# jedisct1/zig-lz4

Measured on AMD Instinct MI355X. Metric: GiB/s uncompressed, block compress+decompress, higher is better.
Workload: dtype u8

## Files before the change

### zig-lz4_amd/csrc/zlz4_compress_fast.hip

```cpp
#include <cstdlib>

#include "zlz4_device.hpp"
#include "zlz4_launch.hpp"

#ifdef ZLZ4_STAMPS
__device__ unsigned long long g_zlz4_stamps[24];
#define STAMP_DECL unsigned long long st_acc[24] = {0,0,0,0,0,0,0,0,0,0,0,0,0,0,0,0,0,0,0,0,0,0,0,0}; unsigned long long st_last = __builtin_amdgcn_s_memtime();
#define STAMP(i) do { unsigned long long st_now; __builtin_amdgcn_sched_barrier(0); \
                      asm volatile("s_memtime %0\n\ts_waitcnt lgkmcnt(0)" : "=s"(st_now) :: "memory"); \
                      __builtin_amdgcn_sched_barrier(0); st_acc[i] += st_now - st_last; st_last = st_now; } while (0)
#define STAMP_COUNT(i) do { st_acc[i] += 1; } while (0)
#define STAMP_FLUSH do { if (lane == 0) for (int st_k = 0; st_k < 24; st_k++) atomicAdd(&g_zlz4_stamps[st_k], st_acc[st_k]); } while (0)
#else
#define STAMP_DECL
#define STAMP(i)
#define STAMP_COUNT(i)
#define STAMP_FLUSH
#endif

namespace zlz4 {

__device__ __forceinline__ uint32_t hash4(uint32_t seq) { return (seq * kHashMul) >> 20; }

__device__ __forceinline__ uint32_t skip_sum(uint32_t x) {
    const uint32_t q = x >> 6, r = x & 63u;
    return 32u * q * (q - 1u) + q * r;
}

__device__ __forceinline__ int64_t emit_last_literals(uint8_t *dst, uint32_t dst_len, uint32_t op,
                                                       const uint8_t *lit_src, uint32_t lit, uint32_t lane) {
    if (lit == 0) return (int64_t)op;
    const uint32_t nle = ext_len_bytes(lit);
    if ((uint64_t)op + 1u + nle + lit > dst_len) return kErrOutputTooSmall;
    if (lane == 0) dst[op] = (uint8_t)((lit >= 15u ? 15u : lit) << 4);
    if (lit >= 15u) write_ext_len(dst + op + 1u, lit, lane);
    copy_bytes(dst + op + 1u + nle, lit_src, lit, lane);
    return (int64_t)(op + 1u + nle + lit);
}

__device__ __forceinline__ uint32_t extend_match(const uint8_t *__restrict__ src, uint32_t m_pos, uint32_t m_cand,
                                                 uint32_t mlen, uint32_t match_limit, uint32_t src_size,
                                                 uint32_t lane) {
    const uint32_t ip0 = m_pos + kMinMatch, mt0 = m_cand + kMinMatch;
    for (;;) {
        const uint32_t p = ip0 + mlen + lane * 16u;
        uint32_t n = 0;
        if (p < match_limit) n = (match_limit - p) < 16u ? (match_limit - p) : 16u;
        uint32_t d = 0;
        if (n > 0) {
            const uint32_t q = mt0 + mlen + lane * 16u;
            if (p + 16u <= src_size) {
                d = first_diff16(ld128(src + p), ld128(src + q));
                if (d > n) d = n;
            } else {
                while (d < n && src[p + d] == src[q + d]) d++;
            }
        }
        const uint64_t stop = ballot(d < 16u);
        if (stop) {
            const uint32_t sl = first_lane(stop);
            return mlen + sl * 16u + rdlane(d, sl);
        }
        mlen += 1024u;
    }
}

template <typename T, int kTag, bool kSeed = false>
__global__ __launch_bounds__(256) void k_compress_fast(
    const uint8_t *__restrict__ d_in, const uint64_t *__restrict__ d_in_off,
    const uint32_t *__restrict__ d_in_len, uint8_t *__restrict__ d_out,
    const uint64_t *__restrict__ d_out_off, const uint32_t *__restrict__ d_out_cap,
    int64_t *__restrict__ d_result, uint32_t nblocks, uint32_t acceleration, uint32_t max_in_len,
    const uint32_t *d_table_in, const uint32_t *__restrict__ d_table_idx, uint32_t *d_table_out) {
    extern __shared__ __attribute__((aligned(16))) uint8_t lds_raw[];
    const uint32_t lane = threadIdx.x & 63u;
    const uint32_t wave_in_wg = threadIdx.x >> 6;
    const uint32_t blk = rfl(blockIdx.x * (blockDim.x >> 6) + wave_in_wg);
    if (blk >= nblocks) return;
    typedef __attribute__((address_space(3))) volatile T lds_entry;
    typedef __attribute__((address_space(3))) volatile uint8_t lds_tag;
    lds_entry *table = (lds_entry *)lds_raw + wave_in_wg * 4096u;
    lds_tag *tags = (lds_tag *)lds_raw + (blockDim.x >> 6) * 4096u * (uint32_t)sizeof(T) + wave_in_wg * 4096u;
    constexpr uint32_t kPosMask = kTag == 2 ? 0x00FFFFFFu : 0xFFFFFFFFu;

    const uint8_t *src = d_in + d_in_off[blk];
    uint8_t *dst = d_out + d_out_off[blk];
    const uint32_t src_size = rfl(d_in_len[blk]);
    const uint32_t dst_len = rfl(d_out_cap[blk]);

    int64_t res;
    if (src_size > kMaxInput) {
        res = kErrInputTooLarge;
    } else if (src_size > max_in_len) {
        res = kErrInvalidState;
    } else if (src_size == 0) {
        res = 0;
    } else if (src_size < kMfLimit + 1u) {
        res = emit_last_literals(dst, dst_len, 0, src, src_size, lane);
    } else {
        if constexpr (kSeed) {
            const uint32_t L = src_size - kMfLimit;
            const uint32_t tix = d_table_idx ? rfl(d_table_idx[blk]) : blk;
            const u32x4 *seed4 = reinterpret_cast<const u32x4 *>(d_table_in + (uint64_t)tix * 4096u);
            for (uint32_t k = lane; k < 1024u; k += 64u) {
                const u32x4 v = seed4[k];
                uint32_t e[4] = {v.x < L ? v.x : 0u, v.y < L ? v.y : 0u, v.z < L ? v.z : 0u, v.w < L ? v.w : 0u};
                if (kTag == 2) {
                    for (int q = 0; q < 4; q++)
                        if (e[q]) e[q] |= ((ld32(src + e[q]) * kHashMul) >> 12 & 0xFFu) << 24;
                }
                for (int q = 0; q < 4; q++) table[4u * k + q] = (T)e[q];
            }
            __builtin_amdgcn_fence(__ATOMIC_RELEASE, "wavefront");
        } else {
        {
            u32x4 z = {0, 0, 0, 0};
            u32x4 *t4 = reinterpret_cast<u32x4 *>(lds_raw) + wave_in_wg * (4096u * sizeof(T) / 16u);
            const uint32_t n16 = 4096u * sizeof(T) / 16u;
            for (uint32_t k = lane; k < n16; k += 64u) t4[k] = z;
        }
        }
        const uint32_t accel = acceleration < 1u ? 1u : (acceleration > 65537u ? 65537u : acceleration);
        const uint32_t cbase = accel > 64u ? accel : 64u;
        const uint32_t s_cbase = skip_sum(cbase);
        const uint32_t L = src_size - kMfLimit;
        const uint32_t match_limit = src_size - kLastLiterals;
        const uint64_t lane_bit = 1ull << lane;
        const uint64_t lanes_below = lane_bit - 1ull;

        uint32_t anchor = 0, op = 0;
        uint32_t F0 = 1;
        bool has_ins = false;
        bool failed = false;
        STAMP_DECL
        STAMP(0);

        uint32_t guard = 0;

        constexpr bool kRing = sizeof(T) == 2;
        uint32_t rpos = 0x80000000u + 4u * lane;
        uint32_t r0 = 0, r1 = 0, r2 = 0;
        uint32_t ring_lim = 0;
        if constexpr (kRing) asm volatile("v_mov_b32 %0, %1" : "=v"(ring_lim) : "s"(src_size - 4u));
        auto ring_q = [&](uint32_t q) -> uint32_t { return q < ring_lim ? q : ring_lim; };
        auto ring_sel = [&](uint32_t A, uint32_t &ja) -> uint32_t {
            uint32_t rel = rfl(A - rpos);
            if (rel >= 256u) {
                const bool reload = rel >= 512u;
                const uint32_t nb = reload ? (A & ~127u) + 4u * lane : rpos + 256u;
                asm volatile("s_waitcnt vmcnt(0)\n\t"
                             "s_cmpk_lt_u32 %[rel], 0x200\n\t"
                             "s_cbranch_scc1 1f\n\t"
                             "global_load_dword %[r0], %[q0], %[src]\n\t"
                             "global_load_dword %[r1], %[q1], %[src]\n\t"
                             "s_waitcnt vmcnt(0)\n\t"
                             "s_branch 2f\n"
                             "1:\n\t"
                             "v_mov_b32 %[r0], %[r1]\n\t"
                             "v_mov_b32 %[r1], %[r2]\n"
                             "2:\n\t"
                             "global_load_dword %[r2], %[q2], %[src]"
                             : [r0] "+v"(r0), [r1] "+v"(r1), [r2] "+v"(r2)
                             : [rel] "s"(rel), [q0] "v"(ring_q(nb)), [q1] "v"(ring_q(nb + 256u)), [q2] "v"(ring_q(nb + 512u)),
                               [src] "s"(src)
                             : "scc", "memory");
                rpos = nb;
                rel = reload ? A & 127u : rel - 256u;
            }
            ja = ((rel & ~3u) + (((A & 3u) + lane) & ~3u)) & 0xFFu;
            return lane >= (rel >> 2) ? r0 : r1;
        };
#define ZLZ4_SEL_DWORD(sel, ja, K) ((uint32_t)__builtin_amdgcn_ds_bpermute((int)add_wrap_byte<4u * (K)>(ja), (int)(sel)))
        auto ring_fwd = [&](uint32_t sel, uint32_t ja, uint32_t A, uint32_t &hi4) -> u32x4 {
            const uint32_t sh = (A + lane) & 3u;
            const uint32_t w0 = (uint32_t)__builtin_amdgcn_ds_bpermute((int)ja, (int)sel);
            const uint32_t w1 = ZLZ4_SEL_DWORD(sel, ja, 1), w2 = ZLZ4_SEL_DWORD(sel, ja, 2), w3 = ZLZ4_SEL_DWORD(sel, ja, 3);
            hi4 = ZLZ4_SEL_DWORD(sel, ja, 4);
            return u32x4{__builtin_amdgcn_alignbyte(w1, w0, sh), __builtin_amdgcn_alignbyte(w2, w1, sh),
                         __builtin_amdgcn_alignbyte(w3, w2, sh), __builtin_amdgcn_alignbyte(hi4, w3, sh)};
        };
        auto ring_fwd2 = [&](uint32_t sel, uint32_t ja, uint32_t A, uint32_t hi4, u32x4 &f2, u32x4 &f3) {
            const uint32_t sh = (A + lane) & 3u;
            const uint32_t w5 = ZLZ4_SEL_DWORD(sel, ja, 5), w6 = ZLZ4_SEL_DWORD(sel, ja, 6), w7 = ZLZ4_SEL_DWORD(sel, ja, 7);
            const uint32_t w8 = ZLZ4_SEL_DWORD(sel, ja, 8), w9 = ZLZ4_SEL_DWORD(sel, ja, 9), w10 = ZLZ4_SEL_DWORD(sel, ja, 10);
            const uint32_t w11 = ZLZ4_SEL_DWORD(sel, ja, 11), w12 = ZLZ4_SEL_DWORD(sel, ja, 12);
            f2 = u32x4{__builtin_amdgcn_alignbyte(w5, hi4, sh), __builtin_amdgcn_alignbyte(w6, w5, sh),
                       __builtin_amdgcn_alignbyte(w7, w6, sh), __builtin_amdgcn_alignbyte(w8, w7, sh)};
            f3 = u32x4{__builtin_amdgcn_alignbyte(w9, w8, sh), __builtin_amdgcn_alignbyte(w10, w9, sh),
                       __builtin_amdgcn_alignbyte(w11, w10, sh), __builtin_amdgcn_alignbyte(w12, w11, sh)};
        };
#undef ZLZ4_SEL_DWORD
        u32x4 fwd_pf = {0, 0, 0, 0};
        uint32_t sel_pf = 0, ja_pf = 0, hi4_pf = 0;
        uint32_t pf_anchor = 0xFFFFFFFFu;
        while (F0 < L) {
            if (++guard > src_size) { failed = true; break; }
            int32_t ub = -1;

            if (accel == 1u && F0 == anchor + 1u && has_ins && (uint64_t)anchor + 192u < L) {
              bool moved = false;
              bool to_generic = false;
              for (;;) {
                const uint32_t A = anchor;
                const uint32_t pos = A + lane;
                if (kRing && pf_anchor != A) {
                    sel_pf = ring_sel(A, ja_pf);
                    fwd_pf = ring_fwd(sel_pf, ja_pf, A, hi4_pf);
                }
                const uint32_t sel = sel_pf, ja = ja_pf, hi4 = hi4_pf;
                const u32x4 fwd = (kRing || pf_anchor == A) ? fwd_pf : ld128(src + pos);
                const uint32_t prod = fwd.x * kHashMul;
                const uint32_t h = prod >> 20;
                const uint32_t tg = (prod >> 12) & 0xFFu;
                const uint32_t mine = kTag == 2 ? (pos | (tg << 24)) : (uint32_t)(T)pos;
                STAMP(1);
                STAMP_COUNT(16);
                uint32_t told = tg;
                const uint32_t old_e = table[h];
                if (kTag == 1) told = tags[h];
                if (kTag == 2) told = old_e >> 24;
                const uint32_t old = old_e & kPosMask;
                uint64_t okm = ballot(old > 0) & ballot(old + kMaxDist >= pos);
                if (kSeed) okm &= ballot(old < pos);
                if (kTag != 0) okm &= ballot(told == tg);
                const bool old_ok = in_mask(okm);
                u32x4 cold = {0, 0, 0, 0};
                if (old_ok) cold = ld128(src + old);
                constexpr bool kGuess2 = sizeof(T) == 4;
                const uint32_t old12 = kGuess2 ? shfl(old, (lane + 12u) & 63u) : 0u;
                const bool pred2 = kGuess2 && old_ok && lane < 52u && old12 == old + 12u;
                u32x4 f2 = {0, 0, 0, 0}, c2 = f2, f3 = f2, c3 = f2;
                if (pred2) {
                    if (!kRing) { f2 = ld128(src + pos + 16u); f3 = ld128(src + pos + 32u); }
                    c2 = ld128(src + old + 16u); c3 = ld128(src + old + 32u);
                }
                STAMP(3);
                table[h] = (T)mine;
                __builtin_amdgcn_fence(__ATOMIC_RELEASE, "wavefront");
                const uint32_t rb = table[h];
                uint64_t losers = ballot(rb != mine);
                uint64_t grp = lane_bit;
                while (losers) {
                    const uint32_t l = first_lane(losers);
                    const uint32_t hh = rdlane(h, l);
                    const uint64_t same = ballot(h == hh);
                    if (in_mask(same)) grp = same;
                    losers &= ~same;
                }
                STAMP(2);

                const uint64_t vom = okm & ballot(cold.x == fwd.x);
                const bool vo = in_mask(vom);
                uint32_t mlo;
                {
                    const uint32_t x1 = fwd.y ^ cold.y, x2 = fwd.z ^ cold.z, x3 = fwd.w ^ cold.w;
                    const uint32_t xs = x1 ? x1 : (x2 ? x2 : x3);
                    const uint32_t xbase = x1 ? 0u : (x2 ? 4u : 8u);
                    mlo = xs ? xbase + ((uint32_t)__builtin_ctz(xs) >> 3) : 12u;
                }
                const uint64_t need2m = vom & ballot(mlo == 12u);
                const bool need2 = in_mask(need2m);
                if (need2 && !pred2) {
                    if (!kRing) { f2 = ld128(src + pos + 16u); f3 = ld128(src + pos + 32u); }
                    c2 = ld128(src + old + 16u); c3 = ld128(src + old + 32u);
                }
                if (kRing && need2m) ring_fwd2(sel, ja, A, hi4, f2, f3);
                if (need2) {
                    const uint32_t d2 = first_diff16_sel(f2, c2);
                    mlo += d2 == 16u ? 16u + first_diff16_sel(f3, c3) : d2;
                }
                const uint64_t singm = ballot(lane_rank(grp) == 0u);
                const uint64_t lt44 = ballot(mlo < 44u);
                const uint64_t cfast = vom & lt44;
                const uint64_t nsing = ~singm;
                const uint64_t slow = (nsing & ~cfast) | (vom & ~lt44);
                const uint64_t fastm = cfast & singm;
                const uint64_t stopm = slow | (cfast & nsing);
                uint32_t J, S;
                {
                    const uint64_t mj = fastm >> lane, ms = stopm >> lane;
                    J = mj ? lane + (uint32_t)__builtin_ctzll(mj) : 64u;
                    S = ms ? lane + (uint32_t)__builtin_ctzll(ms) : 64u;
                }
                const uint32_t v_end = lane + kMinMatch + mlo;
                uint32_t mlo_e = mlo, off_e = pos - old;
                const uint32_t X = J < S ? J : S;
                const uint32_t Q = (mlo << 2) | (in_mask(nsing) ? 2u : 0u) | (vo ? 1u : 0u);
                uint32_t PK;
                {
                    const uint32_t ve_j = shfl(v_end, J & 63u);
                    const bool fastok = J < S;
                    PK = fastok ? (J | ((ve_j + 1u) << 6) | (ve_j >= 63u ? 0x80000000u : 0u)) : 0xFFFFFFFFu;
                }

                STAMP(6);
                uint32_t f = 1;
                uint32_t a = 0;
                uint64_t cov_acc = 0;
                bool continue_generic = false;
                const bool tight = dst_len - op < 512u;
                uint32_t a0 = a;
                uint64_t mm_run = 0;
                uint64_t E_run = 0;
                auto covered_now = [&]() -> uint64_t { return cov_acc | (E_run - (mm_run << 1)); };
                auto flush_run = [&]() {
                    STAMP(9); STAMP_COUNT(21);
                    const uint64_t covm = E_run - (mm_run << 1);
                    const uint64_t ends = (E_run | (1ull << a0) | 1ull) & (lanes_below | lane_bit);
                    const uint32_t pend = 63u - (uint32_t)__builtin_clzll(ends);
                    const bool is_m = in_mask(mm_run);
                    const uint32_t jlast = 63u - (uint32_t)__builtin_clzll(mm_run);
                    const uint64_t litmask = ((1ull << jlast) - 1ull) & ~((1ull << a0) - 1ull) & ~(covm | mm_run);
                    const bool is_lit = in_mask(litmask);
                    const uint64_t extm = mm_run & ballot(mlo_e >= 15u);
                    const uint64_t at_or_above = mm_run & ~lanes_below;
                    const uint32_t my_m = at_or_above ? (uint32_t)__builtin_ctzll(at_or_above) : lane;
                    const uint64_t ownm = ballot(my_m - pend >= 15u);
                    const uint32_t own_l = in_mask(ownm) ? 1u : 0u;
                    const uint64_t lextm = mm_run & ownm;
                    const uint32_t k = lane_rank(mm_run);
                    const uint32_t lb = lane_rank(litmask);
                    const uint32_t o1 = op + 3u * k + lb + 1u + lane_rank(extm) + lane_rank(lextm) + own_l;
                    if (is_lit) dst[o1] = (uint8_t)fwd.x;
                    if (is_m) {
                        const uint32_t lit_k = lane - pend;
                        uint8_t *tk = dst + (o1 - 1u - lit_k - own_l);
                        tk[0] = (uint8_t)(((lit_k < 15u ? lit_k : 15u) << 4) | (mlo_e < 15u ? mlo_e : 15u));
                        if (own_l) tk[1] = (uint8_t)(lit_k - 15u);
                        const uint16_t off16 = (uint16_t)off_e;
                        __builtin_memcpy(dst + o1, &off16, 2);
                        if (mlo_e >= 15u) dst[o1 + 2u] = (uint8_t)(mlo_e - 15u);
                    }
                    const uint32_t nm = (uint32_t)__popcll(mm_run);
                    op += 3u * nm + (uint32_t)__popcll(litmask) + (uint32_t)__popcll(extm) + (uint32_t)__popcll(lextm);
                    cov_acc |= covm;
                    mm_run = 0;
                    E_run = 0;
                    STAMP(10);
                };
                for (;;) {
                    if (mm_run == 0) a0 = a;
                    if (!tight && f < 64u) {
                        uint32_t t_pk, t_j;
#define ZLZ4_FAST_RUN_TRIP                                   \
                            "v_readlane_b32 %[pk], %[PK], %[f]\n\t" \
                            "s_cmp_lt_i32 %[pk], 0\n\t"      \
                            "s_cbranch_scc1 3f\n\t"          \
                            "s_lshr_b32 %[f], %[pk], 6\n\t"  \
                            "s_and_b32 %[j], %[pk], 63\n\t"  \
                            "s_bitset1_b64 %[mm], %[j]\n\t"  \
                            "s_sub_u32 %[a], %[f], 1\n\t"    \
                            "s_bitset1_b64 %[er], %[a]\n\t"
                        asm volatile(
                            "s_nop 3\n"
                            "1:\n\t"
                            ZLZ4_FAST_RUN_TRIP
                            ZLZ4_FAST_RUN_TRIP
                            "s_branch 1b\n"
                            "3:\n"
                            : [f] "+s"(f), [a] "+s"(a), [mm] "+s"(mm_run), [er] "+s"(E_run), [pk] "=&s"(t_pk), [j] "=&s"(t_j)
                            : [PK] "v"(PK)
                            : "scc");
#undef ZLZ4_FAST_RUN_TRIP
                        if (t_pk != 0xFFFFFFFFu) {
                            mm_run |= 1ull << (t_pk & 63u);
                            f = (t_pk >> 6) & 127u;
                            a = f - 1u;
                            if (a == 63u) E_run |= 1ull << 63;
                        }
                    }
                    STAMP(8);
                    if (f >= 64u) {
                        if (a == 0u) continue_generic = true;
                        break;
                    }

                    const uint32_t x = rdlane(X, f);
                    if (x >= 64u) {
                        if (a == 0u) continue_generic = true;
                        break;
                    }
                    const uint32_t q = rdlane(Q, x);
                    uint64_t pm = 0;
                    if (q & 2u) {
                        const uint64_t grp_x = (uint64_t)rdlane((uint32_t)grp, x) | ((uint64_t)rdlane((uint32_t)(grp >> 32), x) << 32);
                        pm = grp_x & ~covered_now() & ((1ull << x) - 1ull);
                    }
                    const uint32_t j = x;
                    const uint32_t m_pos = A + j;
                    uint32_t m_cand, mlen;
                    if (pm) {
                        const uint32_t pr = 63u - (uint32_t)__builtin_clzll(pm);
                        if (rdlane(fwd.x, pr) != rdlane(fwd.x, x)) { STAMP_COUNT(19); STAMP(9); f = x + 1u; continue; }
                        STAMP_COUNT(18);
                        m_cand = A + pr;
                        const uint64_t xa = ((uint64_t)(rdlane(fwd.z, j) ^ rdlane(fwd.z, pr)) << 32) | (rdlane(fwd.y, j) ^ rdlane(fwd.y, pr));
                        const uint32_t xb = rdlane(fwd.w, j) ^ rdlane(fwd.w, pr);
                        if (xa) mlen = (uint32_t)__builtin_ctzll(xa) >> 3;
                        else if (xb) mlen = 8u + ((uint32_t)__builtin_ctz(xb) >> 3);
                        else mlen = extend_match(src, m_pos, m_cand, 12u, match_limit, src_size, lane);
                    } else {
                        if (!(q & 1u)) { STAMP_COUNT(19); STAMP(9); f = x + 1u; continue; }
                        STAMP_COUNT(18);
                        mlen = q >> 2;
                        if (mlen < 44u && !tight) {
                            mm_run |= 1ull << j;
                            a = j + kMinMatch + mlen;
                            if (a < 64u) E_run |= 1ull << a;
                            STAMP(9);
                            if (a >= 64u) break;
                            f = a + 1u;
                            continue;
                        }
                        m_cand = rdlane(old, x);
                        if (mlen >= 44u) mlen = extend_match(src, m_pos, m_cand, 44u, match_limit, src_size, lane);
                    }
                    const uint32_t lit = j - a;
                    const uint32_t offset = m_pos - m_cand;
                    const uint32_t e = j + kMinMatch + mlen;
                    if (!tight && mlen < 270u) {
                        mlo_e = wrlane(mlen, j, mlo_e);
                        off_e = wrlane(offset, j, off_e);
                        mm_run |= 1ull << j;
                        if (e < 64u) E_run |= 1ull << e;
                        a = e;
                        STAMP(9);
                        if (e >= 64u) break;
                        f = e + 1u;
                        continue;
                    }
                    if (mm_run) flush_run();
                    const uint32_t nle = ext_len_bytes(lit), nme = ext_len_bytes(mlen);
                    const uint64_t seq_end = (uint64_t)op + 1u + nle + lit + 2u + nme;
                    if (seq_end > dst_len) { failed = true; break; }
                    if (lane == 0)
                        dst[op] = (uint8_t)(((lit >= 15u ? 15u : lit) << 4) | (mlen >= 15u ? 15u : mlen));
                    if (lit >= 15u) write_ext_len(dst + op + 1u, lit, lane);
                    uint8_t *o = dst + op + 1u + nle;
                    if (lane >= a && lane < j) o[lane - a] = (uint8_t)fwd.x;
                    o += lit;
                    if (lane < 2u) o[lane] = (uint8_t)(offset >> (8u * lane));
                    if (mlen >= 15u) write_ext_len(o + 2u, mlen, lane);
                    op = (uint32_t)seq_end;
                    {
                        const uint64_t upto_e = e >= 64u ? ~0ull : (1ull << e) - 1ull;
                        cov_acc |= upto_e & ~((2ull << j) - 1ull);
                    }
                    a = e;
                    if (e >= 64u) break;
                    f = e + 1u;
                }
                const bool next_win = !continue_generic && !failed && a != 0u && (uint64_t)A + a + 192u < L;
                if (next_win) {
                    pf_anchor = A + a;
                    if constexpr (kRing) {
                        sel_pf = ring_sel(pf_anchor, ja_pf);
                        fwd_pf = ring_fwd(sel_pf, ja_pf, pf_anchor, hi4_pf);
                    } else {
                        fwd_pf = ld128(src + pf_anchor + lane);
                    }
                }
                if (mm_run && !failed) flush_run();
                anchor = A + a;
                STAMP(4);
                const uint32_t f_end = continue_generic ? 64u : (a >= 64u ? 64u : a + 1u);
                const uint64_t ins = ~cov_acc & (f_end >= 64u ? ~0ull : (1ull << f_end) - 1ull);
                if (failed) break;
                const uint64_t gi = grp & ins;
                const bool put_mine = in_mask(ins) && (gi & ~lanes_below & ~lane_bit) == 0;
                if (put_mine || gi == 0) table[h] = (T)(put_mine ? mine : old_e);
                if (kTag == 1 && put_mine) tags[h] = (uint8_t)tg;
                __builtin_amdgcn_fence(__ATOMIC_RELEASE, "wavefront");
                STAMP(5);
                moved = anchor != A;
                to_generic = continue_generic;
                if (next_win) {
                    has_ins = true;
                    F0 = anchor + 1u;
                    continue;
                }
                break;
              }
                if (failed) break;
                if (!to_generic && moved) {
                    if (anchor < L) { has_ins = true; F0 = anchor + 1u; }
                    else { has_ins = false; F0 = L; }
                    continue;
                }
                if (to_generic) ub = 63;
            }

            bool found = false, bailed = false;
            uint32_t m_pos = 0, m_cand = 0, m_local = 0;
            bool m_local_done = false;
            for (;;) {
                const int32_t u = ub + (int32_t)lane;
                uint32_t pos, step_next;
                if (u <= 0) {
                    pos = (u < 0) ? F0 - 1u : F0;
                    step_next = accel;
                } else if (u == 1) {
                    pos = F0 + accel;
                    step_next = accel >> 6;
                } else {
                    const uint32_t x = cbase + (uint32_t)u - 1u;
                    pos = F0 + accel + skip_sum(x) - s_cbase;
                    step_next = x >> 6;
                }
                const bool is_probe = u >= 0;
                const bool bail = is_probe && ((uint64_t)pos + step_next > L);
                const uint64_t bail_mask = ballot(bail);
                const uint32_t nb = bail_mask ? first_lane(bail_mask) : 64u;
                const bool active = (lane < nb) && (is_probe || has_ins);

                const bool have16 = active && (pos + 16u <= src_size);
                u32x4 fwd = {0, 0, 0, 0};
                if (have16) fwd = ld128(src + pos);
                else if (active) fwd.x = ld32(src + pos);
                const uint32_t prod = fwd.x * kHashMul;
                const uint32_t h = prod >> 20;
                const uint32_t tg = (prod >> 12) & 0xFFu;
                const uint32_t mine = kTag == 2 ? (pos | (tg << 24)) : (uint32_t)(T)pos;

                uint32_t old_e = 0, rb = 0, told = tg;
                if (active) {
                    old_e = table[h];
                    if (kTag == 1) told = tags[h];
                    table[h] = (T)mine;
                }
                if (kTag == 2) told = old_e >> 24;
                const uint32_t old = old_e & kPosMask;
                __builtin_amdgcn_fence(__ATOMIC_RELEASE, "wavefront");
                if (active) rb = table[h];
                uint64_t losers = ballot(active && rb != mine);
                uint64_t grp = lane_bit;
                int32_t pred = -1;
                while (losers) {
                    const uint32_t l = first_lane(losers);
                    const uint32_t hh = rdlane(h, l);
                    const uint64_t same = ballot(active && h == hh);
                    if (active && h == hh) {
                        grp = same;
                        const uint64_t below = same & lanes_below;
                        pred = below ? 63 - (int32_t)__clzll((long long)below) : -1;
                    }
                    losers &= ~same;
                }
                const uint32_t pred_pos = shfl(pos, (uint32_t)(pred < 0 ? 0 : pred));
                const uint32_t cand = pred >= 0 ? pred_pos : old;

                bool valid = is_probe && active && cand > 0 && cand < pos && (cand + kMaxDist >= pos) &&
                             (kTag == 0 || pred >= 0 || told == tg);
                u32x4 cnd = {0, 0, 0, 0};
                if (valid) {
                    if (have16) cnd = ld128(src + cand); else cnd.x = ld32(src + cand);
                    valid = cnd.x == fwd.x;
                }
                const uint64_t valid_mask = ballot(valid);

                if (valid_mask) {
                    const uint32_t wl = first_lane(valid_mask);
                    if (active && lane > wl) table[h] = (T)old_e;
                    __builtin_amdgcn_fence(__ATOMIC_RELEASE, "wavefront");
                    const uint64_t upto = (2ull << wl) - 1ull;
                    if (active && lane <= wl && ((grp & upto & ~lanes_below & ~lane_bit) == 0)) {
                        table[h] = (T)mine;
                        if (kTag == 1) tags[h] = (uint8_t)tg;
                    }
                    uint32_t loc = 0;
                    bool loc_done = false;
                    if (lane == wl) {
                        const uint32_t lim = match_limit - (pos + kMinMatch);
                        if (have16) {
                            u32x4 a = fwd, b = cnd;
                            a.x = 0; b.x = 0;
                            loc = first_diff16(a, b) - 4u;
                            if (loc >= lim) { loc = lim; loc_done = true; }
                            else if (loc < 12u) loc_done = true;
                        }
                    }
                    m_pos = rdlane(pos, wl);
                    m_cand = rdlane(cand, wl);
                    m_local = rdlane(loc, wl);
                    m_local_done = rdlane((uint32_t)loc_done, wl) != 0;
                    found = true;
                    break;
                }
                if (bail_mask) {
                    if constexpr (kSeed) {
                        if (active && ((grp & ~lanes_below & ~lane_bit) == 0) && grp != lane_bit) table[h] = (T)mine;
                        __builtin_amdgcn_fence(__ATOMIC_RELEASE, "wavefront");
                    }
                    bailed = true; break;
                }
                if (active && ((grp & ~lanes_below & ~lane_bit) == 0)) {
                    if (grp != lane_bit) table[h] = (T)mine;
                    if (kTag == 1) tags[h] = (uint8_t)tg;
                }
                __builtin_amdgcn_fence(__ATOMIC_RELEASE, "wavefront");
                ub += 64;
            }
            if (bailed || !found) break;
            STAMP_COUNT(20);

            const uint32_t mlen = m_local_done ? m_local
                                               : extend_match(src, m_pos, m_cand, m_local, match_limit, src_size, lane);

            const uint32_t lit = m_pos - anchor;
            const uint32_t nle = ext_len_bytes(lit), nme = ext_len_bytes(mlen);
            const uint64_t seq_end = (uint64_t)op + 1u + nle + lit + 2u + nme;
            if (seq_end > dst_len) { failed = true; break; }
            if (lane == 0)
                dst[op] = (uint8_t)(((lit >= 15u ? 15u : lit) << 4) | (mlen >= 15u ? 15u : mlen));
            if (lit >= 15u) write_ext_len(dst + op + 1u, lit, lane);
            uint8_t *o = dst + op + 1u + nle;
            copy_bytes(o, src + anchor, lit, lane);
            o += lit;
            const uint32_t offset = m_pos - m_cand;
            if (lane < 2u) o[lane] = (uint8_t)(offset >> (8u * lane));
            if (mlen >= 15u) write_ext_len(o + 2u, mlen, lane);
            op = (uint32_t)seq_end;

            const uint32_t end = m_pos + kMinMatch + mlen;
            anchor = end;
            if (end < L) { has_ins = true; F0 = end + 1u; }
            else { has_ins = false; F0 = L; }
        }
        if constexpr (kRing) asm volatile("s_waitcnt vmcnt(0)" : "+v"(r2));
        if constexpr (kSeed) {
            if (!failed && has_ins && F0 >= L && lane == 0) {
                const uint32_t prod = ld32(src + anchor) * kHashMul;
                table[prod >> 20] = (T)(kTag == 2 ? (anchor | ((prod >> 12 & 0xFFu) << 24)) : anchor);
            }
        }
        res = failed ? kErrOutputTooSmall
                     : emit_last_literals(dst, dst_len, op, src + anchor, src_size - anchor, lane);
        STAMP(7);
        STAMP_FLUSH;
    }
    if constexpr (kSeed) {
        if (d_table_out) {
            const uint32_t tix = d_table_idx ? rfl(d_table_idx[blk]) : blk;
            const uint32_t *seed = d_table_in + (uint64_t)tix * 4096u;
            uint32_t *out = d_table_out + (uint64_t)blk * 4096u;
            const bool merged = src_size >= kMfLimit + 1u && src_size <= max_in_len && src_size <= kMaxInput && res >= 0;
            if (merged) {
                const uint32_t L = src_size - kMfLimit;
                __builtin_amdgcn_fence(__ATOMIC_RELEASE, "wavefront");
                for (uint32_t k = lane; k < 4096u; k += 64u) {
                    const uint32_t v = seed[k];
                    const uint32_t loaded = v < L ? v : 0u;
                    const uint32_t f = (uint32_t)table[k] & kPosMask;
                    out[k] = f != loaded ? f : v;
                }
            } else if (out != seed) {
                const u32x4 *s4 = reinterpret_cast<const u32x4 *>(seed);
                u32x4 *o4 = reinterpret_cast<u32x4 *>(out);
                for (uint32_t k = lane; k < 1024u; k += 64u) o4[k] = s4[k];
            }
        }
    }
    if (lane == 0) d_result[blk] = res;
}

__global__ __launch_bounds__(256) void k_load_dict(const uint8_t *__restrict__ d_dict, const uint64_t *__restrict__ d_dict_off,
                                                   const uint32_t *__restrict__ d_dict_len, uint32_t *__restrict__ d_tables,
                                                   int64_t *__restrict__ d_result, uint32_t ndicts) {
    __shared__ uint32_t t[4096];
    const uint32_t d = blockIdx.x;
    if (d >= ndicts) return;
    const uint32_t lane = threadIdx.x & 63u;
    const uint32_t len = d_dict_len[d];
    const uint32_t size = len < 65536u ? len : 65536u;
    const uint8_t *tail = d_dict + d_dict_off[d] + (len - size);
    for (uint32_t k = threadIdx.x; k < 4096u; k += blockDim.x) t[k] = 0;
    __syncthreads();
    if (size >= kMinMatch) {
        const uint32_t n = size - kMinMatch;
        for (uint32_t base = threadIdx.x - lane; base < n; base += blockDim.x) {
            const uint32_t i = base + lane;
            const bool act = i < n;
            const uint32_t h = act ? hash4(ld32(tail + i)) : 0xFFFFFFFFu;
            const uint32_t hr = shfl(h, lane + 1u);
            if (act && !(lane < 63u && hr == h)) atomicMax(&t[h], i);
        }
    }
    __syncthreads();
    uint32_t *out = d_tables + (uint64_t)d * 4096u;
    for (uint32_t k = threadIdx.x; k < 4096u; k += blockDim.x) out[k] = t[k];
    if (threadIdx.x == 0) d_result[d] = (int64_t)size;
}

}

extern "C" int zlz4_launch_compress_fast(hipStream_t stream, const uint8_t *d_in, const uint64_t *d_in_off,
                                         const uint32_t *d_in_len, uint8_t *d_out, const uint64_t *d_out_off,
                                         const uint32_t *d_out_cap, int64_t *d_result, uint32_t nblocks,
                                         uint32_t max_in_len, uint32_t acceleration) {
    if (nblocks == 0) return 0;
    static const uint32_t lds_pad = [] { const char *e = zlz4_tune_env("ZLZ4_TUNE_LDS_PAD"); return e ? (uint32_t)atoi(e) : 0u; }();
    static const uint32_t tune_wpw = [] { const char *e = zlz4_tune_env("ZLZ4_TUNE_WPW"); return e ? (uint32_t)atoi(e) : 0u; }();
    static const int tune_tag = [] { const char *e = zlz4_tune_env("ZLZ4_TUNE_TAG"); return e ? atoi(e) : -1; }();
#define ZLZ4_LAUNCH_FAST(KERN, T, TAG, WPW, LDS)                                                                      \
    hipLaunchKernelGGL((zlz4::KERN<T, TAG>), dim3((nblocks + (WPW) - 1) / (WPW)), dim3(64 * (WPW)), (LDS),              \
                       stream, d_in, d_in_off, d_in_len, d_out, d_out_off, d_out_cap, d_result, nblocks, acceleration,  \
                       max_in_len, nullptr, nullptr, nullptr)
    if (max_in_len <= 65536u + 11u) {
        const uint32_t wpw = (tune_wpw == 2 || tune_wpw == 4) ? tune_wpw : 1;
        if (tune_tag > 0) ZLZ4_LAUNCH_FAST(k_compress_fast, uint16_t, 1, wpw, wpw * (4096 * sizeof(uint16_t) + 4096) + lds_pad);
        else ZLZ4_LAUNCH_FAST(k_compress_fast, uint16_t, 0, wpw, wpw * 4096 * sizeof(uint16_t) + lds_pad);
    } else {
        const uint32_t wpw = (tune_wpw == 2) ? 2 : 1;
        if (tune_tag != 0 && max_in_len <= (1u << 24)) ZLZ4_LAUNCH_FAST(k_compress_fast, uint32_t, 2, wpw, wpw * 4096 * sizeof(uint32_t) + lds_pad);
        else ZLZ4_LAUNCH_FAST(k_compress_fast, uint32_t, 0, wpw, wpw * 4096 * sizeof(uint32_t) + lds_pad);
    }
#undef ZLZ4_LAUNCH_FAST
    return zlz4_launch_status();
}

extern "C" int zlz4_launch_compress_fast_continue(hipStream_t stream, const uint8_t *d_in, const uint64_t *d_in_off,
                                                  const uint32_t *d_in_len, uint8_t *d_out, const uint64_t *d_out_off,
                                                  const uint32_t *d_out_cap, const uint32_t *d_table_in,
                                                  const uint32_t *d_table_idx, uint32_t *d_table_out, int64_t *d_result,
                                                  uint32_t nblocks, uint32_t max_in_len, uint32_t acceleration) {
    if (nblocks == 0) return 0;
    static const int tune_tag = [] { const char *e = zlz4_tune_env("ZLZ4_TUNE_TAG"); return e ? atoi(e) : -1; }();
#define ZLZ4_LAUNCH_SEEDED(T, TAG)                                                                                      \
    hipLaunchKernelGGL((zlz4::k_compress_fast<T, TAG, true>), dim3(nblocks), dim3(64), 4096 * sizeof(T), stream, d_in,   \
                       d_in_off, d_in_len, d_out, d_out_off, d_out_cap, d_result, nblocks, acceleration, max_in_len,      \
                       d_table_in, d_table_idx, d_table_out)
    if (max_in_len <= 65536u + 11u) ZLZ4_LAUNCH_SEEDED(uint16_t, 0);
    else if (tune_tag != 0 && max_in_len <= (1u << 24)) ZLZ4_LAUNCH_SEEDED(uint32_t, 2);
    else ZLZ4_LAUNCH_SEEDED(uint32_t, 0);
#undef ZLZ4_LAUNCH_SEEDED
    return zlz4_launch_status();
}

extern "C" int zlz4_launch_load_dict(hipStream_t stream, const uint8_t *d_dict, const uint64_t *d_dict_off,
                                     const uint32_t *d_dict_len, uint32_t *d_tables, int64_t *d_result, uint32_t ndicts) {
    if (ndicts == 0) return 0;
    hipLaunchKernelGGL(zlz4::k_load_dict, dim3(ndicts), dim3(256), 0, stream, d_dict, d_dict_off, d_dict_len, d_tables,
                       d_result, ndicts);
    return zlz4_launch_status();
}

#ifdef ZLZ4_STAMPS
extern "C" int zlz4_debug_read_stamps(unsigned long long *out16, int reset) {
    if (hipMemcpyFromSymbol(out16, HIP_SYMBOL(g_zlz4_stamps), 24 * sizeof(unsigned long long)) != hipSuccess) return ZLZ4_ERR_DEVICE;
    if (reset) {
        unsigned long long z[24] = {0};
        if (hipMemcpyToSymbol(HIP_SYMBOL(g_zlz4_stamps), z, sizeof z) != hipSuccess) return ZLZ4_ERR_DEVICE;
    }
    return 0;
}
#endif
```

Baseline: 92.24.

## Stage compressor input ring window in LDS instead of register ds_bpermute gathers

Replaces the register-resident three-dword ring, which was read through many ds_bpermute cross-lane shuffles, with a 576-byte per-wave LDS ring buffer. Global loads are written into LDS, including a mirrored head region so reads can wrap, and forward windows are then read with one b32 plus one unaligned 128-bit LDS load per 16 bytes. This is meant to cut the number of permute instructions per window probe and to free VGPRs. In exchange it adds ds_writes, a wavefront fence and extra LDS per wave, and the static_assert is there to keep the occupancy granule count unchanged.

```diff
diff --git a/zig-lz4_amd/csrc/zlz4_compress_fast.hip b/zig-lz4_amd/csrc/zlz4_compress_fast.hip
--- a/zig-lz4_amd/csrc/zlz4_compress_fast.hip
+++ b/zig-lz4_amd/csrc/zlz4_compress_fast.hip
@@ -65,6 +65,10 @@
     }
 }
 
+constexpr uint32_t kRingBytes = 576;
+constexpr uint32_t kLdsGranule = 1280;
+static_assert(4096 * sizeof(uint16_t) + kRingBytes <= 7 * kLdsGranule, "the ring must fit the granules the u16 table already occupies");
+
 template <typename T, int kTag, bool kSeed = false>
 __global__ __launch_bounds__(256) void k_compress_fast(
     const uint8_t *__restrict__ d_in, const uint64_t *__restrict__ d_in_off,
@@ -138,60 +142,58 @@
         uint32_t guard = 0;
 
         constexpr bool kRing = sizeof(T) == 2;
+        typedef __attribute__((address_space(3))) const volatile uint8_t lds_ring_byte;
+        lds_ring_byte *ring = (lds_ring_byte *)lds_raw +
+                              (blockDim.x >> 6) * (4096u * (uint32_t)sizeof(T) + (kTag == 1 ? 4096u : 0u)) + wave_in_wg * kRingBytes;
         uint32_t rpos = 0x80000000u + 4u * lane;
-        uint32_t r0 = 0, r1 = 0, r2 = 0;
+        uint32_t r2 = 0;
         uint32_t ring_lim = 0;
         if constexpr (kRing) asm volatile("v_mov_b32 %0, %1" : "=v"(ring_lim) : "s"(src_size - 4u));
         auto ring_q = [&](uint32_t q) -> uint32_t { return q < ring_lim ? q : ring_lim; };
-        auto ring_sel = [&](uint32_t A, uint32_t &ja) -> uint32_t {
-            uint32_t rel = rfl(A - rpos);
+        const uint32_t ring_addr = (uint32_t)(uintptr_t)ring;
+        auto ring_move = [&](uint32_t A) {
+            const uint32_t rel = rfl(A - rpos);
             if (rel >= 256u) {
                 const bool reload = rel >= 512u;
                 const uint32_t nb = reload ? (A & ~127u) + 4u * lane : rpos + 256u;
+                const uint32_t i0 = nb & 511u, i1 = (nb + 256u) & 511u;
+                uint32_t t0;
                 asm volatile("s_waitcnt vmcnt(0)\n\t"
                              "s_cmpk_lt_u32 %[rel], 0x200\n\t"
                              "s_cbranch_scc1 1f\n\t"
-                             "global_load_dword %[r0], %[q0], %[src]\n\t"
-                             "global_load_dword %[r1], %[q1], %[src]\n\t"
+                             "global_load_dword %[t0], %[q0], %[src]\n\t"
+                             "global_load_dword %[r2], %[q1], %[src]\n\t"
                              "s_waitcnt vmcnt(0)\n\t"
-                             "s_branch 2f\n"
+                             "ds_write_b32 %[a0], %[t0]\n\t"
+                             "ds_write_b32 %[m0], %[t0]\n"
                              "1:\n\t"
-                             "v_mov_b32 %[r0], %[r1]\n\t"
-                             "v_mov_b32 %[r1], %[r2]\n"
-                             "2:\n\t"
+                             "ds_write_b32 %[a1], %[r2]\n\t"
+                             "ds_write_b32 %[m1], %[r2]\n\t"
                              "global_load_dword %[r2], %[q2], %[src]"
-                             : [r0] "+v"(r0), [r1] "+v"(r1), [r2] "+v"(r2)
+                             : [r2] "+v"(r2), [t0] "=&v"(t0)
                              : [rel] "s"(rel), [q0] "v"(ring_q(nb)), [q1] "v"(ring_q(nb + 256u)), [q2] "v"(ring_q(nb + 512u)),
+                               [a0] "v"(ring_addr + i0), [m0] "v"(ring_addr + (i0 < 64u ? i0 + 512u : i0)),
+                               [a1] "v"(ring_addr + i1), [m1] "v"(ring_addr + (i1 < 64u ? i1 + 512u : i1)),
                                [src] "s"(src)
                              : "scc", "memory");
                 rpos = nb;
-                rel = reload ? A & 127u : rel - 256u;
+                __builtin_amdgcn_fence(__ATOMIC_RELEASE, "wavefront");
             }
-            ja = ((rel & ~3u) + (((A & 3u) + lane) & ~3u)) & 0xFFu;
-            return lane >= (rel >> 2) ? r0 : r1;
         };
-#define ZLZ4_SEL_DWORD(sel, ja, K) ((uint32_t)__builtin_amdgcn_ds_bpermute((int)add_wrap_byte<4u * (K)>(ja), (int)(sel)))
-        auto ring_fwd = [&](uint32_t sel, uint32_t ja, uint32_t A, uint32_t &hi4) -> u32x4 {
+        typedef u32x4 u32x4_a4 __attribute__((aligned(4)));
+        typedef __attribute__((address_space(3))) const volatile u32x4_a4 lds_ring_16;
+        typedef __attribute__((address_space(3))) const volatile uint32_t lds_ring_4;
+        uint32_t ring_hi = 0;
+        auto ring_rd = [&](uint32_t A, uint32_t K) -> u32x4 {
+            lds_ring_byte *b = ring + ((A + lane) & 508u) + K;
             const uint32_t sh = (A + lane) & 3u;
-            const uint32_t w0 = (uint32_t)__builtin_amdgcn_ds_bpermute((int)ja, (int)sel);
-            const uint32_t w1 = ZLZ4_SEL_DWORD(sel, ja, 1), w2 = ZLZ4_SEL_DWORD(sel, ja, 2), w3 = ZLZ4_SEL_DWORD(sel, ja, 3);
-            hi4 = ZLZ4_SEL_DWORD(sel, ja, 4);
-            return u32x4{__builtin_amdgcn_alignbyte(w1, w0, sh), __builtin_amdgcn_alignbyte(w2, w1, sh),
-                         __builtin_amdgcn_alignbyte(w3, w2, sh), __builtin_amdgcn_alignbyte(hi4, w3, sh)};
+            const uint32_t lo = K == 0u ? *(lds_ring_4 *)b : ring_hi;
+            const u32x4 w = *(lds_ring_16 *)(b + 4u);
+            ring_hi = w.w;
+            return u32x4{__builtin_amdgcn_alignbyte(w.x, lo, sh), __builtin_amdgcn_alignbyte(w.y, w.x, sh),
+                         __builtin_amdgcn_alignbyte(w.z, w.y, sh), __builtin_amdgcn_alignbyte(w.w, w.z, sh)};
         };
-        auto ring_fwd2 = [&](uint32_t sel, uint32_t ja, uint32_t A, uint32_t hi4, u32x4 &f2, u32x4 &f3) {
-            const uint32_t sh = (A + lane) & 3u;
-            const uint32_t w5 = ZLZ4_SEL_DWORD(sel, ja, 5), w6 = ZLZ4_SEL_DWORD(sel, ja, 6), w7 = ZLZ4_SEL_DWORD(sel, ja, 7);
-            const uint32_t w8 = ZLZ4_SEL_DWORD(sel, ja, 8), w9 = ZLZ4_SEL_DWORD(sel, ja, 9), w10 = ZLZ4_SEL_DWORD(sel, ja, 10);
-            const uint32_t w11 = ZLZ4_SEL_DWORD(sel, ja, 11), w12 = ZLZ4_SEL_DWORD(sel, ja, 12);
-            f2 = u32x4{__builtin_amdgcn_alignbyte(w5, hi4, sh), __builtin_amdgcn_alignbyte(w6, w5, sh),
-                       __builtin_amdgcn_alignbyte(w7, w6, sh), __builtin_amdgcn_alignbyte(w8, w7, sh)};
-            f3 = u32x4{__builtin_amdgcn_alignbyte(w9, w8, sh), __builtin_amdgcn_alignbyte(w10, w9, sh),
-                       __builtin_amdgcn_alignbyte(w11, w10, sh), __builtin_amdgcn_alignbyte(w12, w11, sh)};
-        };
-#undef ZLZ4_SEL_DWORD
         u32x4 fwd_pf = {0, 0, 0, 0};
-        uint32_t sel_pf = 0, ja_pf = 0, hi4_pf = 0;
         uint32_t pf_anchor = 0xFFFFFFFFu;
         while (F0 < L) {
             if (++guard > src_size) { failed = true; break; }
@@ -204,10 +206,9 @@
                 const uint32_t A = anchor;
                 const uint32_t pos = A + lane;
                 if (kRing && pf_anchor != A) {
-                    sel_pf = ring_sel(A, ja_pf);
-                    fwd_pf = ring_fwd(sel_pf, ja_pf, A, hi4_pf);
-                }
-                const uint32_t sel = sel_pf, ja = ja_pf, hi4 = hi4_pf;
+                    ring_move(A);
+                    fwd_pf = ring_rd(A, 0u);
+                }
                 const u32x4 fwd = (kRing || pf_anchor == A) ? fwd_pf : ld128(src + pos);
                 const uint32_t prod = fwd.x * kHashMul;
                 const uint32_t h = prod >> 20;
@@ -264,7 +265,7 @@
                     if (!kRing) { f2 = ld128(src + pos + 16u); f3 = ld128(src + pos + 32u); }
                     c2 = ld128(src + old + 16u); c3 = ld128(src + old + 32u);
                 }
-                if (kRing && need2m) ring_fwd2(sel, ja, A, hi4, f2, f3);
+                if (kRing && need2m) { f2 = ring_rd(A, 16u); f3 = ring_rd(A, 32u); }
                 if (need2) {
                     const uint32_t d2 = first_diff16_sel(f2, c2);
                     mlo += d2 == 16u ? 16u + first_diff16_sel(f3, c3) : d2;
@@ -454,8 +455,8 @@
                 if (next_win) {
                     pf_anchor = A + a;
                     if constexpr (kRing) {
-                        sel_pf = ring_sel(pf_anchor, ja_pf);
-                        fwd_pf = ring_fwd(sel_pf, ja_pf, pf_anchor, hi4_pf);
+                        ring_move(pf_anchor);
+                        fwd_pf = ring_rd(pf_anchor, 0u);
                     } else {
                         fwd_pf = ld128(src + pf_anchor + lane);
                     }
@@ -707,8 +708,9 @@
                        max_in_len, nullptr, nullptr, nullptr)
     if (max_in_len <= 65536u + 11u) {
         const uint32_t wpw = (tune_wpw == 2 || tune_wpw == 4) ? tune_wpw : 1;
-        if (tune_tag > 0) ZLZ4_LAUNCH_FAST(k_compress_fast, uint16_t, 1, wpw, wpw * (4096 * sizeof(uint16_t) + 4096) + lds_pad);
-        else ZLZ4_LAUNCH_FAST(k_compress_fast, uint16_t, 0, wpw, wpw * 4096 * sizeof(uint16_t) + lds_pad);
+        const uint32_t ring = wpw * zlz4::kRingBytes;
+        if (tune_tag > 0) ZLZ4_LAUNCH_FAST(k_compress_fast, uint16_t, 1, wpw, wpw * (4096 * sizeof(uint16_t) + 4096) + ring + lds_pad);
+        else ZLZ4_LAUNCH_FAST(k_compress_fast, uint16_t, 0, wpw, wpw * 4096 * sizeof(uint16_t) + ring + lds_pad);
     } else {
         const uint32_t wpw = (tune_wpw == 2) ? 2 : 1;
         if (tune_tag != 0 && max_in_len <= (1u << 24)) ZLZ4_LAUNCH_FAST(k_compress_fast, uint32_t, 2, wpw, wpw * 4096 * sizeof(uint32_t) + lds_pad);
@@ -726,7 +728,8 @@
     if (nblocks == 0) return 0;
     static const int tune_tag = [] { const char *e = zlz4_tune_env("ZLZ4_TUNE_TAG"); return e ? atoi(e) : -1; }();
 #define ZLZ4_LAUNCH_SEEDED(T, TAG)                                                                                      \
-    hipLaunchKernelGGL((zlz4::k_compress_fast<T, TAG, true>), dim3(nblocks), dim3(64), 4096 * sizeof(T), stream, d_in,   \
+    hipLaunchKernelGGL((zlz4::k_compress_fast<T, TAG, true>), dim3(nblocks), dim3(64),                                   \
+                       4096 * sizeof(T) + (sizeof(T) == 2 ? zlz4::kRingBytes : 0u), stream, d_in,                         \
                        d_in_off, d_in_len, d_out, d_out_off, d_out_cap, d_result, nblocks, acceleration, max_in_len,      \
                        d_table_in, d_table_idx, d_table_out)
     if (max_in_len <= 65536u + 11u) ZLZ4_LAUNCH_SEEDED(uint16_t, 0);
```

Result: no change. 92.80 (median of 6 runs) (+0.6%).
